# GATB/dsk

Measured on AMD Instinct MI355X. Metric: distinct k-mers counted/sec (whole node), k=31, higher is better.
Workload: dtype u64

## Files before the change

### dsk_amd/csrc/engine.h

```cpp
#pragma once
#include <algorithm>
#include <cstring>
#include <string>
#include <vector>

#include "../../include/dskgpu.h"
#include "layouts.h"

hipError_t placed_malloc(void** out, size_t bytes);

struct DevBuf {
    void* p = nullptr;
    size_t cap = 0;
    hipError_t ensure(size_t bytes) {
        if (bytes <= cap) return hipSuccess;
        size_t want = ((p ? bytes + bytes / 16 : bytes) + 255) & ~size_t(255);
        if (p) { (void)hipFree(p); p = nullptr; cap = 0; }
        hipError_t e = placed_malloc(&p, want);
        if (e == hipSuccess) cap = want; else p = nullptr;
        return e;
    }
    int ensure_keep(size_t bytes, size_t keep, hipStream_t stream) {
        if (bytes <= cap) return 0;
        void* np = nullptr;
        size_t want = ((std::max(bytes, cap + cap / 2) + 255) & ~size_t(255));
        if (hipMalloc(&np, want) != hipSuccess) return -1;
        if (keep && p) {
            if (hipMemcpyAsync(np, p, keep, hipMemcpyDeviceToDevice, stream) != hipSuccess || hipStreamSynchronize(stream) != hipSuccess) { (void)hipFree(np); return -1; }
        }
        if (p) (void)hipFree(p);
        p = np; cap = want;
        return 0;
    }
    void release() { if (p) (void)hipFree(p); p = nullptr; cap = 0; }
    template <class T> T* as() const { return reinterpret_cast<T*>(p); }
};

enum Scalar { SC_NCH1 = 0, SC_MLEN1, SC_NCH2, SC_MLEN2, SC_OVERFLOW, SC_F, SC_SORTFLAG, SC_OVF2, SC_OVF1, SC_RSLEN, SC_RSWORK, SC_RSWORK2, SC_RSTIES, SC_EXT, SC_NCHAINED, SC_NCH_S, SC_MLEN_S, SC_WORK2, SC_COUNT = 24 };

struct Stage { const char* name; hipEvent_t ev; };

struct Tuning {
    bool no_opt1 = false, no_opt2 = false;
    bool no_aligned = false;
    u32 rs_heavy = 0;
    u32 rs_bbits = 0;
    u32 rs_block_rows = 0;
    bool sk_exact = false, no_recsrc = false;
    u32 opt_cap = 0;
    u64 opt_slice = 0;
    u64 sk_slice = 0, sk_minslice = 2000;
    u32 table_maxload = 0;
    long long max_ext = -1;
    bool no_sample = false;
    bool no_heavy = false;
    bool verbose = false;
    bool no_level0 = false; u32 l0_passes = 0;
    u64 rs_max_rows = 0;
    u32 ps_maxc = 0;
    bool sk_generic = false;
    bool l0_keys = false;
    u32 mp_pass_mkeys = 0;
    u64 rs_slab_rows = 0;
    bool unitig_stages = false;
    bool cc_plain = false, cc_stages = false;
    bool correct_staged = false;
    void read() {
        auto on = [](const char* n) { return getenv(n) != nullptr; };
        auto num = [](const char* n, u64 dflt) { const char* e = getenv(n); return e ? (u64)atoll(e) : dflt; };
        no_opt1 = on("DSKGPU_NO_OPT1"); no_opt2 = on("DSKGPU_NO_OPT2"); no_aligned = on("DSKGPU_NO_ALIGNED");
        sk_exact = on("DSKGPU_SK_EXACT");
        no_recsrc = on("DSKGPU_NO_RECSRC");
        opt_cap = (u32)num("DSKGPU_OPT_CAP", 0) & ~7u; opt_slice = num("DSKGPU_OPT_SLICE", 0) & ~7ull;
        sk_slice = num("DSKGPU_SK_SLICE", 0); sk_minslice = num("DSKGPU_SK_MINSLICE", 2000);
        table_maxload = (u32)num("DSKGPU_TABLE_MAXLOAD", 0);
        max_ext = getenv("DSKGPU_MAX_EXT") ? atoll(getenv("DSKGPU_MAX_EXT")) : -1;
        no_sample = on("DSKGPU_NO_SAMPLE"); no_heavy = on("DSKGPU_NO_HEAVY"); verbose = on("DSKGPU_VERBOSE"); no_level0 = on("DSKGPU_NO_LEVEL0"); l0_passes = (u32)num("DSKGPU_L0_PASSES", 0); mp_pass_mkeys = (u32)num("DSKGPU_MP_PASS_MKEYS", 0); rs_max_rows = num("DSKGPU_RS_MAX_ROWS", 0); l0_keys = on("DSKGPU_L0_KEYS"); sk_generic = on("DSKGPU_SK_GENERIC"); ps_maxc = (u32)num("DSKGPU_PS_MAXC", 0);
        rs_slab_rows = num("DSKGPU_RS_SLAB_ROWS", 0);
        unitig_stages = on("DSKGPU_UNITIG_STAGES");
        cc_plain = on("DSKGPU_CC_PLAIN"); cc_stages = on("DSKGPU_CC_STAGES");
        correct_staged = on("DSKGPU_CORRECT_STAGED");
        rs_block_rows = (u32)num("DSKGPU_RS_BLOCK_ROWS", 0); rs_bbits = (u32)num("DSKGPU_RS_BBITS", 0); rs_heavy = (u32)num("DSKGPU_RS_HEAVY", 0);
    }
};

struct SparseRows {
    int W = 0;
    const void* keys = nullptr; const u32 *ab = nullptr, *soff = nullptr, *fstart = nullptr; u32 cap = 0, F = 0;
    u64 n_sparse = 0; u32 n_tail = 0; RowsIn tail_w{}; const u32* tail_ab = nullptr;
    template <class S> S as(u32 qpc = 0) const { return S{static_cast<decltype(S::keys)>(keys), ab, soff, fstart, cap, F, qpc}; }
    Rows2C tail2() const { return Rows2C{tail_w.w[1], tail_w.w[0], tail_ab}; }
};

struct PartPasses {
    struct Pass { u64 row_base; u32 nparts, off_index; };
    std::vector<Pass> passes; DevBuf part_off, flag; u32 off_used = 0; bool ok = false; u64 row_base = 0;
    std::vector<u32> h_off;
};

struct RowSort {
    DevBuf fix_list;
    DevBuf g[4];
    DevBuf del, lens;
    std::vector<u64> h_del; std::vector<u32> h_lens, h_lin;
    DevBuf ovs;
    u32 flag = 0, listed = 0;
    u64* hist_pin = nullptr; size_t hist_pin_n = 0;
    bool part_mode = false; u32 n_parts = 0; u32* h_part_off = nullptr; size_t h_part_cap = 0; DevBuf part_off;
    std::vector<u64> h_part_off64;
    PartPasses mp;
    void release() {
        for (DevBuf* b : {&fix_list, &g[0], &g[1], &g[2], &g[3], &del, &lens, &ovs, &part_off, &mp.part_off, &mp.flag}) b->release();
        if (hist_pin) (void)hipHostFree(hist_pin);
        if (h_part_off) (void)hipHostFree(h_part_off);
        hist_pin = nullptr; h_part_off = nullptr;
    }
};

struct Query {
    DevBuf table, packed, inval, deg;
    u64 cap = 0;
    bool valid = false;
    void release() { table.release(); packed.release(); inval.release(); deg.release(); cap = 0; valid = false; }
    void invalidate() { valid = false; }
};

struct Components {
    DevBuf comp, first, cols;
    dskgpu_component_stats stats{};
    bool valid = false;
    void release() { for (DevBuf* b : {&comp, &first, &cols}) b->release(); stats = dskgpu_component_stats{}; valid = false; }
// ... 237 lines not shown
```

### dsk_amd/csrc/partsort.h

```cpp
#pragma once
#include "rowsort.h"
#include "rowsort2.h"

#ifndef PS_NT
#define PS_NT 1024
#define PS_RPT 4
#endif
#define PS_CAP (PS_NT * PS_RPT)
#define PS_BINS 4096
#define PS_MAXC 4096u
#define PS_MAXQ 512

struct PsParams { u32 qpp, nparts_sparse; int sh; u32 n_tail, maxc; };

__global__ __launch_bounds__(PS_NT) void k_part_sort(RsSparse s, const u64* __restrict__ tail_k, const u32* __restrict__ tail_v, PsParams pp,
                                                     u64* __restrict__ ov, u32* __restrict__ oab, u32* __restrict__ part_off, u32* __restrict__ flag) {
    __shared__ u64 lk[PS_CAP];
    __shared__ u32 la[PS_CAP];
    __shared__ u32 cnt[PS_BINS];
    __shared__ u32 lsoff[PS_MAXQ + 1];
    __shared__ u32 wsum[PS_NT / 64 + 1];
    const u32 tid = threadIdx.x, lane = tid & 63, wave = tid >> 6;
    const u32 p = blockIdx.x;
    const bool is_tail = p >= pp.nparts_sparse;
    const u32 q0 = is_tail ? s.F : p * pp.qpp, q1 = is_tail ? s.F : (q0 + pp.qpp < s.F ? q0 + pp.qpp : s.F), nq = q1 - q0;
    for (u32 x = tid; x <= nq; x += PS_NT) lsoff[x] = s.soff[q0 + x];
    for (u32 b = tid; b < PS_BINS; b += PS_NT) cnt[b] = 0;
    __syncthreads();
    const u32 r0 = is_tail ? s.soff[s.F] : lsoff[0];
    const u32 n = is_tail ? pp.n_tail : lsoff[nq] - r0;
    if (tid == 0) {
        part_off[p] = r0;
        if (p + 1 == gridDim.x) part_off[p + 1] = r0 + n;
    }
    if (n > PS_CAP) {
        if (tid == 0) *flag = 1u;
        for (u32 i = tid; i < n; i += PS_NT) {
            const u32 r = r0 + i;
            if (is_tail) { ov[(u64)r] = tail_k[i]; oab[(u64)r] = tail_v[i]; }
            else {
                u32 lo = 0, hi = nq;
                while (hi - lo > 1) { const u32 mid = (lo + hi) >> 1; if (lsoff[mid] <= r) lo = mid; else hi = mid; }
                const u64 src = rs_sp_base(s, q0 + lo) + (u64)(r - lsoff[lo]);
                ov[(u64)r] = kunmix(s.keys[src]); oab[(u64)r] = s.ab[src];
            }
        }
        return;
    }
    if (n == 0) return;
    u64 k[PS_RPT]; u32 a[PS_RPT], rb[PS_RPT];
#pragma unroll
    for (int j = 0; j < PS_RPT; ++j) {
        const u32 i = tid + (u32)j * PS_NT;
        const u32 r = r0 + (i < n ? i : n - 1);
        if (is_tail) { k[j] = tail_k[r - r0]; a[j] = tail_v[r - r0]; }
        else {
            u32 lo = 0, hi = nq;
            while (hi - lo > 1) { const u32 mid = (lo + hi) >> 1; if (lsoff[mid] <= r) lo = mid; else hi = mid; }
            const u64 src = rs_sp_base(s, q0 + lo) + (u64)(r - lsoff[lo]);
            k[j] = kunmix(s.keys[src]); a[j] = s.ab[src];
        }
    }
#pragma unroll
    for (int j = 0; j < PS_RPT; ++j) {
        const u32 i = tid + (u32)j * PS_NT;
        u32 bin = (u32)(k[j] >> pp.sh); bin = bin < PS_BINS ? bin : PS_BINS - 1;
        rb[j] = i < n ? (bin << 16) | atomicAdd(&cnt[bin], 1u) : 0xFFFFFFFFu;
    }
    __syncthreads();
    {
        constexpr int CPT = PS_BINS / PS_NT;
        u32 c[CPT], sum = 0;
#pragma unroll
        for (int x = 0; x < CPT; ++x) { c[x] = cnt[tid * CPT + x]; sum += c[x]; }
        const u32 inc = wave_incl_scan(sum);
        if (lane == 63) wsum[wave] = inc;
        __syncthreads();
        u32 run = inc - sum;
#pragma unroll
        for (int x = 0; x < PS_NT / 64; ++x) { const u32 v = wsum[x]; if ((u32)x < wave) run += v; }
        bool heavy = false;
#pragma unroll
        for (int x = 0; x < CPT; ++x) { cnt[tid * CPT + x] = (run << 16) | c[x]; run += c[x]; heavy = heavy || c[x] > pp.maxc; }
        if (heavy) *flag = 1u;
    }
    __syncthreads();
    u32 pos[PS_RPT], cb[PS_RPT];
#pragma unroll
    for (int j = 0; j < PS_RPT; ++j) {
        pos[j] = 0; cb[j] = 0;
        if (rb[j] != 0xFFFFFFFFu) {
            cb[j] = cnt[rb[j] >> 16];
            pos[j] = (cb[j] >> 16) + (rb[j] & 0xFFFFu);
            lk[pos[j]] = k[j]; la[pos[j]] = a[j];
        }
    }
    __syncthreads();
    bool moved = false;
#pragma unroll
    for (int j = 0; j < PS_RPT; ++j) {
        const u32 c = cb[j] & 0xFFFFu;
        if (rb[j] != 0xFFFFFFFFu && c > 1u && c <= PS_MAXC) {
            const u32 o = cb[j] >> 16;
            u32 less = 0;
            for (u32 x = 0; x < c; ++x) less += lk[o + x] < k[j] ? 1u : 0u;
            pos[j] = o + less; moved = true;
        }
    }
    __syncthreads();
    if (moved) {
#pragma unroll
        for (int j = 0; j < PS_RPT; ++j)
            if (rb[j] != 0xFFFFFFFFu && (cb[j] & 0xFFFFu) > 1u && (cb[j] & 0xFFFFu) <= PS_MAXC) { lk[pos[j]] = k[j]; la[pos[j]] = a[j]; }
    }
    __syncthreads();
    for (u32 i = tid; i < n; i += PS_NT) { ov[(u64)r0 + i] = lk[i]; oab[(u64)r0 + i] = la[i]; }
}

#ifndef PS2_RPT
#define PS2_RPT 2
#endif
#define PS2_CAP (PS_NT * PS2_RPT)
__device__ __forceinline__ u32 ps2_bin(u64 hi, u64 lo, int sh) {
    const u64 v = sh >= 64 ? hi >> (sh - 64) : sh == 0 ? lo : ((hi << (64 - sh)) | (lo >> sh));
    return v < PS_BINS ? (u32)v : PS_BINS - 1;
}
__global__ __launch_bounds__(PS_NT) void k_part_sort2(Rs2Sparse s, Rows2C tail, PsParams pp, Rows2 o, u32* __restrict__ part_off, u32* __restrict__ flag) {
    __shared__ u64 lh[PS2_CAP];
    __shared__ u64 ll[PS2_CAP];
    __shared__ u32 la[PS2_CAP];
    __shared__ u32 cnt[PS_BINS];
    __shared__ u32 lsoff[PS_MAXQ + 1];
    __shared__ u32 wsum[PS_NT / 64 + 1];
    const u32 tid = threadIdx.x, lane = tid & 63, wave = tid >> 6;
    const u32 p = blockIdx.x;
    const bool is_tail = p >= pp.nparts_sparse;
    const u32 q0 = is_tail ? s.F : p * pp.qpp, q1 = is_tail ? s.F : (q0 + pp.qpp < s.F ? q0 + pp.qpp : s.F), nq = q1 - q0;
    for (u32 x = tid; x <= nq; x += PS_NT) lsoff[x] = s.soff[q0 + x];
    for (u32 b = tid; b < PS_BINS; b += PS_NT) cnt[b] = 0;
    __syncthreads();
    const u32 r0 = is_tail ? s.soff[s.F] : lsoff[0];
    const u32 n = is_tail ? pp.n_tail : lsoff[nq] - r0;
    if (tid == 0) {
        part_off[p] = r0;
        if (p + 1 == gridDim.x) part_off[p + 1] = r0 + n;
    }
    if (n > PS2_CAP) {
        if (tid == 0) *flag = 1u;
        for (u32 i = tid; i < n; i += PS_NT) {
            const u32 r = r0 + i;
            if (is_tail) { const u64 th = tail.hi[i], tl = tail.lo[i]; const u32 ta = tail.ab[i]; o.hi[(u64)r] = th; o.lo[(u64)r] = tl; o.ab[(u64)r] = ta; }
            else {
                u32 lo = 0, hi = nq;
                while (hi - lo > 1) { const u32 mid = (lo + hi) >> 1; if (lsoff[mid] <= r) lo = mid; else hi = mid; }
                const u64 src = rs2_sp_base(s, q0 + lo) + (u64)(r - lsoff[lo]);
                K2 kx = s.keys[src]; kunmixN(kx);
                o.hi[(u64)r] = kx.w[1]; o.lo[(u64)r] = kx.w[0]; o.ab[(u64)r] = s.ab[src];
            }
        }
        return;
    }
    if (n == 0) return;
    u64 kh[PS2_RPT], kl[PS2_RPT]; u32 a[PS2_RPT], rb[PS2_RPT];
#pragma unroll
    for (int j = 0; j < PS2_RPT; ++j) {
        const u32 i = tid + (u32)j * PS_NT;
        const u32 r = r0 + (i < n ? i : n - 1);
        if (is_tail) { kh[j] = tail.hi[r - r0]; kl[j] = tail.lo[r - r0]; a[j] = tail.ab[r - r0]; }
        else {
            u32 lo = 0, hi = nq;
            while (hi - lo > 1) { const u32 mid = (lo + hi) >> 1; if (lsoff[mid] <= r) lo = mid; else hi = mid; }
            const u64 src = rs2_sp_base(s, q0 + lo) + (u64)(r - lsoff[lo]);
            K2 kx = s.keys[src]; kunmixN(kx);
            kh[j] = kx.w[1]; kl[j] = kx.w[0]; a[j] = s.ab[src];
        }
    }
#pragma unroll
    for (int j = 0; j < PS2_RPT; ++j) {
        const u32 i = tid + (u32)j * PS_NT;
        const u32 bin = ps2_bin(kh[j], kl[j], pp.sh);
        rb[j] = i < n ? (bin << 16) | atomicAdd(&cnt[bin], 1u) : 0xFFFFFFFFu;
    }
    __syncthreads();
    {
        constexpr int CPT = PS_BINS / PS_NT;
        u32 c[CPT], sum = 0;
#pragma unroll
        for (int x = 0; x < CPT; ++x) { c[x] = cnt[tid * CPT + x]; sum += c[x]; }
        const u32 inc = wave_incl_scan(sum);
        if (lane == 63) wsum[wave] = inc;
        __syncthreads();
        u32 run = inc - sum;
#pragma unroll
        for (int x = 0; x < PS_NT / 64; ++x) { const u32 v = wsum[x]; if ((u32)x < wave) run += v; }
        bool heavy = false;
#pragma unroll
        for (int x = 0; x < CPT; ++x) { cnt[tid * CPT + x] = (run << 16) | c[x]; run += c[x]; heavy = heavy || c[x] > pp.maxc; }
        if (heavy) *flag = 1u;
    }
    __syncthreads();
    u32 pos[PS2_RPT], cb[PS2_RPT];
#pragma unroll
    for (int j = 0; j < PS2_RPT; ++j) {
        pos[j] = 0; cb[j] = 0;
        if (rb[j] != 0xFFFFFFFFu) {
            cb[j] = cnt[rb[j] >> 16];
            pos[j] = (cb[j] >> 16) + (rb[j] & 0xFFFFu);
            lh[pos[j]] = kh[j]; ll[pos[j]] = kl[j]; la[pos[j]] = a[j];
        }
    }
    __syncthreads();
    bool moved = false;
#pragma unroll
    for (int j = 0; j < PS2_RPT; ++j) {
        const u32 c = cb[j] & 0xFFFFu;
        if (rb[j] != 0xFFFFFFFFu && c > 1u && c <= PS_MAXC) {
            const u32 ob = cb[j] >> 16;
            u32 less = 0;
            for (u32 x = 0; x < c; ++x) { const u64 h = lh[ob + x], l = ll[ob + x]; less += (h < kh[j] || (h == kh[j] && l < kl[j])) ? 1u : 0u; }
            pos[j] = ob + less; moved = true;
        }
    }
    __syncthreads();
    if (moved) {
#pragma unroll
        for (int j = 0; j < PS2_RPT; ++j)
            if (rb[j] != 0xFFFFFFFFu && (cb[j] & 0xFFFFu) > 1u && (cb[j] & 0xFFFFu) <= PS_MAXC) { lh[pos[j]] = kh[j]; ll[pos[j]] = kl[j]; la[pos[j]] = a[j]; }
    }
    __syncthreads();
    for (u32 i = tid; i < n; i += PS_NT) { o.hi[(u64)r0 + i] = lh[i]; o.lo[(u64)r0 + i] = ll[i]; o.ab[(u64)r0 + i] = la[i]; }
}

#define PS4_CAP PS_NT
__device__ __forceinline__ u64 rs4_sp_base(const Rs4Sparse& s, u32 q) { return s.cap ? (u64)q * s.cap : (u64)s.fstart[q]; }
__device__ __forceinline__ u32 ps4_bin(u64 w0, u64 w1, u64 w2, u64 w3, int sh) {
    const int wi = sh >> 6, b = sh & 63;
    const u64 lo = wi == 0 ? w0 : wi == 1 ? w1 : wi == 2 ? w2 : w3;
    const u64 hi = wi == 0 ? w1 : wi == 1 ? w2 : wi == 2 ? w3 : 0ull;
    const u64 v = b ? (lo >> b) | (hi << (64 - b)) : lo;
    return v < PS_BINS ? (u32)v : PS_BINS - 1;
}
__global__ __launch_bounds__(PS_NT) void k_part_sort4(Rs4Sparse s, PsParams pp, RowsOut o, u32* oab, u32* part_off, u32* flag) {
    __shared__ u64 lw[4][PS4_CAP];
    __shared__ u32 la[PS4_CAP];
    __shared__ u32 cnt[PS_BINS];
    __shared__ u32 lsoff[PS_MAXQ + 1];
    __shared__ u32 wsum[PS_NT / 64 + 1];
    const u32 tid = threadIdx.x, lane = tid & 63, wave = tid >> 6;
    const u32 p = blockIdx.x;
    const u32 q0 = p * pp.qpp < s.F ? p * pp.qpp : s.F, q1 = q0 + pp.qpp < s.F ? q0 + pp.qpp : s.F, nq = q1 - q0;
    for (u32 x = tid; x <= nq; x += PS_NT) lsoff[x] = s.soff[q0 + x];
    for (u32 b = tid; b < PS_BINS; b += PS_NT) cnt[b] = 0;
    __syncthreads();
    const u32 r0 = lsoff[0];
    const u32 n = lsoff[nq] - r0;
    if (tid == 0) {
        part_off[p] = r0;
        if (p + 1 == gridDim.x) part_off[p + 1] = r0 + n;
    }
    if (n > PS4_CAP) {
        if (tid == 0) *flag = 1u;
        for (u32 i = tid; i < n; i += PS_NT) {
            const u32 r = r0 + i;
            u32 lo = 0, hi = nq;
            while (hi - lo > 1) { const u32 mid = (lo + hi) >> 1; if (lsoff[mid] <= r) lo = mid; else hi = mid; }
            const u64 src = rs4_sp_base(s, q0 + lo) + (u64)(r - lsoff[lo]);
            KN<4> kx;
#pragma unroll
            for (int x = 0; x < 4; ++x) kx.w[x] = s.keys[src].w[x];
            kunmixN(kx);
#pragma unroll
            for (int x = 0; x < 4; ++x) o.w[x][(u64)r] = kx.w[x];
            oab[(u64)r] = s.ab[src];
        }
        return;
    }
    if (n == 0) return;
    const bool have = tid < n;
    u64 k0, k1, k2, k3; u32 a;
    {
        const u32 r = r0 + (have ? tid : n - 1);
        u32 lo = 0, hi = nq;
        while (hi - lo > 1) { const u32 mid = (lo + hi) >> 1; if (lsoff[mid] <= r) lo = mid; else hi = mid; }
// ... 56 lines not shown
```

### dsk_amd/csrc/rowsort.hip

```cpp
#include <cstdio>
#include <vector>

#include "engine.h"
#include "partsort.h"

#include <rocprim/device/device_radix_sort.hpp>

namespace {

__global__ void k_set_rs_scalars(u32* __restrict__ sc4, u32 len, u32 nwords, u32* __restrict__ z0 = nullptr, u32* __restrict__ z1 = nullptr) {
    if (threadIdx.x == 0) sc4[0] = len;
    else if (threadIdx.x < nwords) sc4[threadIdx.x] = 0u;
    if (threadIdx.x == 32 && z0) *z0 = 0u;
    if (threadIdx.x == 33 && z1) *z1 = 0u;
}
__global__ void k_sort_back(const u32* __restrict__ sc, const u32* __restrict__ ovs, u64* __restrict__ out) {
    if (threadIdx.x == 0) { out[0] = sc[SC_SORTFLAG]; out[1] = ovs ? ovs[0] : 0u; }
}
#ifndef SORT_TOP_BITS
#define SORT_TOP_BITS 32u
#endif

template <class T>
int grow_pinned(dskgpu_ctx* ctx, T*& p, size_t& cap, size_t need, size_t alloc) {
// ... 531 lines not shown
                { const int e2 = rows2_rounds(ctx, r2, s2); if (e2) return e2; }
            }
            lib = ctx->rs.flag != 0;
        }
        if (lib && m >= 0xFFFF0000ull) return fail(ctx, DSKGPU_E_OVERFLOW, "row sort: one value range of the >= 2^32 rows holds 2^32 rows itself (not a k-mer spectrum)");
        if (lib && W == 2) {
            const u64* src[2] = {T.lo + b, T.hi + b};
            { const int rc = sort_index_multiword(ctx, src, m, 2); if (rc) return rc; }
            const unsigned gb = (unsigned)((m + 255) / 256);
            const u32* idx = ctx->srt_idx.as<u32>();
            hipLaunchKernelGGL(k_gather<u64>, dim3(gb), dim3(256), 0, ctx->stream, K.lo + b, (const u64*)(T.lo + b), idx, m);
            hipLaunchKernelGGL(k_gather<u64>, dim3(gb), dim3(256), 0, ctx->stream, K.hi + b, (const u64*)(T.hi + b), idx, m);
            hipLaunchKernelGGL(k_gather<u32>, dim3(gb), dim3(256), 0, ctx->stream, K.ab + b, (const u32*)(T.ab + b), idx, m);
            CKL("row sort: group gather");
            CK(hipMemcpyAsync(T.lo + b, K.lo + b, m * 8, hipMemcpyDeviceToDevice, ctx->stream));
            CK(hipMemcpyAsync(T.hi + b, K.hi + b, m * 8, hipMemcpyDeviceToDevice, ctx->stream));
            CK(hipMemcpyAsync(T.ab + b, K.ab + b, m * 4, hipMemcpyDeviceToDevice, ctx->stream));
            CK(hipStreamSynchronize(ctx->stream));
            ctx->stats.sort_fallback = 1; ++nlib;
        } else if (lib) {
            size_t tmp = 0;
            const unsigned end_bit = (unsigned)(total - sb);
            CK(rocprim::radix_sort_pairs(nullptr, tmp, tk + b, k + b, tv + b, v + b, (size_t)m, 0u, end_bit, ctx->stream));
            CK(ctx->srt_tmp.ensure(tmp));
            CK(rocprim::radix_sort_pairs(ctx->srt_tmp.p, tmp, tk + b, k + b, tv + b, v + b, (size_t)m, 0u, end_bit, ctx->stream));
            CK(hipMemcpyAsync(tk + b, k + b, m * 8, hipMemcpyDeviceToDevice, ctx->stream));
            CK(hipMemcpyAsync(tv + b, v + b, m * 4, hipMemcpyDeviceToDevice, ctx->stream));
            CK(hipStreamSynchronize(ctx->stream));
            ctx->stats.sort_fallback = 1; ++nlib;
        }
    }
    if (ctx->tune.verbose) fprintf(stderr, "[dskgpu] row sort: %llu rows (>= 2^32 path) in %u slab(s), %u group(s) on their top %d bits, %u through the library sort\n", (unsigned long long)n, S, ngroups, sb, nlib);
    ctx->rs.flag = 0; ctx->rs.listed = 0;
    if (W == 1) { ctx->res_w[0] = tk; ctx->res_ab = tv; }
    else { ctx->res_w[1] = T.hi; ctx->res_w[0] = T.lo; ctx->res_ab = T.ab; }
    return DSKGPU_OK;
}

}

static u64 part_sort_cap(int W) { return W == 1 ? PS_CAP : W == 2 ? PS2_CAP : PS4_CAP; }
static u32 part_sort_qpp(int W, u64 F, u64 n_sparse) {
    const u64 mean = std::max<u64>(1, (n_sparse + F - 1) / std::max<u64>(F, 1));
    return (u32)std::min<u64>(std::max<u64>(1, (part_sort_cap(W) * 3 / 4) / mean), PS_MAXQ);
}
u32 part_sort_nparts(const SparseRows& rows) {
    const u32 qpp = part_sort_qpp(rows.W, rows.F, rows.n_sparse);
    return (u32)((rows.F + qpp - 1) / qpp) + (rows.n_tail ? 1u : 0u);
}
int launch_part_sort(dskgpu_ctx* ctx, const SparseRows& rows, RowsOut out, u32* out_ab, u32* d_part_off, u32* d_flag, u32* nparts_out) {
    const int W = rows.W;
    const u32 qpp = part_sort_qpp(W, rows.F, rows.n_sparse), nparts = part_sort_nparts(rows), nps = nparts - (rows.n_tail ? 1u : 0u);
    const int sh = std::max(0, 2 * (int)ctx->cfg.kmer_size - 12);
    const PsParams pp{qpp, nps, W == 1 ? std::min(sh, 52) : sh, rows.n_tail, ctx->tune.ps_maxc ? std::min<u32>(ctx->tune.ps_maxc, PS_MAXC) : PS_MAXC};
    if (W == 1) hipLaunchKernelGGL(k_part_sort, dim3(nparts), dim3(PS_NT), 0, ctx->stream, rows.as<RsSparse>(), rows.tail_w.w[0], rows.tail_ab, pp, out.w[0], out_ab, d_part_off, d_flag);
    else if (W == 2) hipLaunchKernelGGL(k_part_sort2, dim3(nparts), dim3(PS_NT), 0, ctx->stream, rows.as<Rs2Sparse>(), rows.tail2(), pp, Rows2{out.w[1], out.w[0], out_ab}, d_part_off, d_flag);
    else hipLaunchKernelGGL(k_part_sort4, dim3(nparts), dim3(PS_NT), 0, ctx->stream, rows.as<Rs4Sparse>(), pp, out, out_ab, d_part_off, d_flag);
    CKL("k_part_sort");
    *nparts_out = nparts;
    return DSKGPU_OK;
}

namespace {

int sort_rows_partition_order(dskgpu_ctx* ctx, const SparseRows& rows, u64 n, Round* r) {
    const int W = rows.W;
    const u32 nparts = part_sort_nparts(rows);
    DevBuf* dst_w = W == 4 ? ctx->out_w : ctx->srt_w;
    DevBuf& dst_ab = W == 4 ? ctx->out_ab : ctx->srt_ab;
    for (int x = 0; x < W; ++x) CK(dst_w[x].ensure(n * 8));
    CK(dst_ab.ensure(n * 4));
    CK(ctx->rs.part_off.ensure(((size_t)nparts + 2) * 4));
    { const int rc = grow_pinned(ctx, ctx->rs.h_part_off, ctx->rs.h_part_cap, (size_t)nparts + 2, ((size_t)nparts + 2) * 2); if (rc) return rc; }
    u32* sc = ctx->scalars.as<u32>();
    hipLaunchKernelGGL(k_set_rs_scalars, dim3(1), dim3(64), 0, ctx->stream, sc + SC_RSLEN, 0u, 1u, sc + SC_SORTFLAG, (u32*)nullptr);
    u32 np = 0;
    RowsOut out{};
    for (int x = 0; x < W; ++x) out.w[x] = dst_w[x].as<u64>();
    { const int rc = launch_part_sort(ctx, rows, out, dst_ab.as<u32>(), ctx->rs.part_off.as<u32>(), sc + SC_SORTFLAG, &np); if (rc) return rc; }
    CK(hipMemcpyAsync(ctx->rs.h_part_off, ctx->rs.part_off.p, ((size_t)nparts + 1) * 4, hipMemcpyDeviceToHost, ctx->stream));
    ctx->rs.part_mode = true; ctx->rs.n_parts = nparts; ctx->rs.h_part_off64.clear();
    r->back = 2;
    for (int x = 0; x < W; ++x) ctx->res_w[x] = dst_w[x].as<u64>();
    ctx->res_ab = dst_ab.as<u32>();
    return DSKGPU_OK;
}

int sort_rows4(dskgpu_ctx* ctx, u64 n, Round* r) {
    constexpr int W = 4;
    CK(ctx->srt_k.ensure(n * 8)); CK(ctx->s_val.ensure(n * 8));
    CK(ctx->srt_idx.ensure(n * 4)); CK(ctx->srt_idx2.ensure(n * 4));
    const unsigned gb = (unsigned)((n + 255) / 256);
    RowsIn ri{}; RowsOut ro{};
    for (int x = 0; x < W; ++x) { CK(ctx->srt_w[x].ensure(n * 8)); ri.w[x] = ctx->out_w[x].as<u64>(); ro.w[x] = ctx->srt_w[x].as<u64>(); }
    const int bits = 2 * (int)ctx->cfg.kmer_size;
    const bool msd = n <= RS_MAX_ROWS;
    u64* aos = nullptr;
    if (msd) {
        CK(ctx->srt_k2.ensure(n * 8 * (size_t)AosRow<W>::WORDS));
        aos = ctx->srt_k2.as<u64>();
        hipLaunchKernelGGL(k_top_key_aos<W>, dim3(gb), dim3(256), 0, ctx->stream, ri, ctx->out_ab.as<u32>(), n, bits, ctx->srt_k.as<u64>(), ctx->srt_idx.as<u32>(), aos);
    } else hipLaunchKernelGGL(k_top_key<W>, dim3(gb), dim3(256), 0, ctx->stream, ri, n, bits, ctx->srt_k.as<u64>(), ctx->srt_idx.as<u32>());
    u32* flag = ctx->scalars.as<u32>() + SC_SORTFLAG;
    const u32* ties = nullptr;
    const u32* idx; const u64* skey; int run_shift;
    if (msd) {
        const int e = msd_sort_pairs(ctx, ctx->srt_k.as<u64>(), ctx->srt_idx.as<u32>(), ctx->s_val.as<u64>(), ctx->srt_idx2.as<u32>(), n, 63);
        if (e) return e;
        CK(hipMemcpyAsync(&ctx->rs.flag, flag, 4, hipMemcpyDeviceToHost, ctx->stream));
// ... 156 lines not shown
```

Measured before the change: 27.02 billion.

## Make partition sort persistent with prefetch of next partition's rows

Converts k_part_sort and k_part_sort2 into persistent kernels launched with a grid of about two blocks per CU. Each block loops over partitions with stride gridDim and double-buffers the segment offsets. The global loads for the next partition are issued while the current one is binned and sorted in shared memory. This targets the load latency that each block previously exposed before any compute, at the cost of more registers, extra synchronisation, and less occupancy-driven latency hiding. A DSKGPU_PS_GRID env knob sets the grid size.

```diff
diff --git a/dsk_amd/csrc/engine.h b/dsk_amd/csrc/engine.h
--- a/dsk_amd/csrc/engine.h
+++ b/dsk_amd/csrc/engine.h
@@ -58,6 +58,7 @@
     bool no_level0 = false; u32 l0_passes = 0;
     u64 rs_max_rows = 0;
     u32 ps_maxc = 0;
+    u32 ps_grid = 0;
     bool sk_generic = false;
     bool l0_keys = false;
     u32 mp_pass_mkeys = 0;
@@ -77,6 +78,7 @@
         max_ext = getenv("DSKGPU_MAX_EXT") ? atoll(getenv("DSKGPU_MAX_EXT")) : -1;
         no_sample = on("DSKGPU_NO_SAMPLE"); no_heavy = on("DSKGPU_NO_HEAVY"); verbose = on("DSKGPU_VERBOSE"); no_level0 = on("DSKGPU_NO_LEVEL0"); l0_passes = (u32)num("DSKGPU_L0_PASSES", 0); mp_pass_mkeys = (u32)num("DSKGPU_MP_PASS_MKEYS", 0); rs_max_rows = num("DSKGPU_RS_MAX_ROWS", 0); l0_keys = on("DSKGPU_L0_KEYS"); sk_generic = on("DSKGPU_SK_GENERIC"); ps_maxc = (u32)num("DSKGPU_PS_MAXC", 0);
         rs_slab_rows = num("DSKGPU_RS_SLAB_ROWS", 0);
+        ps_grid = (u32)std::min<u64>(num("DSKGPU_PS_GRID", 0), 1u << 20);
         unitig_stages = on("DSKGPU_UNITIG_STAGES");
         cc_plain = on("DSKGPU_CC_PLAIN"); cc_stages = on("DSKGPU_CC_STAGES");
         correct_staged = on("DSKGPU_CORRECT_STAGED");
diff --git a/dsk_amd/csrc/partsort.h b/dsk_amd/csrc/partsort.h
--- a/dsk_amd/csrc/partsort.h
+++ b/dsk_amd/csrc/partsort.h
@@ -11,110 +11,153 @@
 #define PS_MAXC 4096u
 #define PS_MAXQ 512
 
-struct PsParams { u32 qpp, nparts_sparse; int sh; u32 n_tail, maxc; };
+struct PsParams { u32 qpp, nparts_sparse; int sh; u32 n_tail, maxc, nblocks; };
 
-__global__ __launch_bounds__(PS_NT) void k_part_sort(RsSparse s, const u64* __restrict__ tail_k, const u32* __restrict__ tail_v, PsParams pp,
+__device__ __forceinline__ u32 ps_q0(const PsParams& pp, u32 F, u32 p) { return p >= pp.nparts_sparse ? F : p * pp.qpp; }
+__device__ __forceinline__ u32 ps_nq(const PsParams& pp, u32 F, u32 p) {
+    if (p >= pp.nparts_sparse) return 0u;
+    const u32 q0 = p * pp.qpp;
+    return (q0 + pp.qpp < F ? q0 + pp.qpp : F) - q0;
+}
+__global__ __launch_bounds__(PS_NT, 8) void k_part_sort(RsSparse s, const u64* __restrict__ tail_k, const u32* __restrict__ tail_v, PsParams pp,
                                                      u64* __restrict__ ov, u32* __restrict__ oab, u32* __restrict__ part_off, u32* __restrict__ flag) {
     __shared__ u64 lk[PS_CAP];
     __shared__ u32 la[PS_CAP];
     __shared__ u32 cnt[PS_BINS];
-    __shared__ u32 lsoff[PS_MAXQ + 1];
+    __shared__ u32 lsoff[2][PS_MAXQ + 1];
     __shared__ u32 wsum[PS_NT / 64 + 1];
     const u32 tid = threadIdx.x, lane = tid & 63, wave = tid >> 6;
-    const u32 p = blockIdx.x;
-    const bool is_tail = p >= pp.nparts_sparse;
-    const u32 q0 = is_tail ? s.F : p * pp.qpp, q1 = is_tail ? s.F : (q0 + pp.qpp < s.F ? q0 + pp.qpp : s.F), nq = q1 - q0;
-    for (u32 x = tid; x <= nq; x += PS_NT) lsoff[x] = s.soff[q0 + x];
+    const u32 G = gridDim.x;
+    u32 p = blockIdx.x;
+    if (p >= pp.nblocks) return;
+    u64 kn[PS_RPT]; u32 an[PS_RPT];
+#pragma unroll
+    for (int j = 0; j < PS_RPT; ++j) { kn[j] = 0; an[j] = 0; }
+    auto fetch = [&](u32 pf, const u32* ls) {
+        const bool tl = pf >= pp.nparts_sparse;
+        const u32 q0 = ps_q0(pp, s.F, pf), nq = ps_nq(pp, s.F, pf);
+        const u32 r0 = ls[0], n = tl ? pp.n_tail : ls[nq] - r0;
+        if (n == 0 || n > PS_CAP) return;
+#pragma unroll
+        for (int j = 0; j < PS_RPT; ++j) {
+            const u32 i = tid + (u32)j * PS_NT;
+            const u32 ii = i < n ? i : n - 1;
+            if (tl) { kn[j] = tail_k[ii]; an[j] = tail_v[ii]; }
+            else {
+                const u32 r = r0 + ii;
+                u32 lo = 0, hi = nq;
+                while (hi - lo > 1) { const u32 mid = (lo + hi) >> 1; if (ls[mid] <= r) lo = mid; else hi = mid; }
+                const u64 src = rs_sp_base(s, q0 + lo) + (u64)(r - ls[lo]);
+                kn[j] = s.keys[src]; an[j] = s.ab[src];
+            }
+        }
+    };
     for (u32 b = tid; b < PS_BINS; b += PS_NT) cnt[b] = 0;
-    __syncthreads();
-    const u32 r0 = is_tail ? s.soff[s.F] : lsoff[0];
-    const u32 n = is_tail ? pp.n_tail : lsoff[nq] - r0;
-    if (tid == 0) {
-        part_off[p] = r0;
-        if (p + 1 == gridDim.x) part_off[p + 1] = r0 + n;
-    }
-    if (n > PS_CAP) {
-        if (tid == 0) *flag = 1u;
-        for (u32 i = tid; i < n; i += PS_NT) {
-            const u32 r = r0 + i;
-            if (is_tail) { ov[(u64)r] = tail_k[i]; oab[(u64)r] = tail_v[i]; }
-            else {
-                u32 lo = 0, hi = nq;
-                while (hi - lo > 1) { const u32 mid = (lo + hi) >> 1; if (lsoff[mid] <= r) lo = mid; else hi = mid; }
-                const u64 src = rs_sp_base(s, q0 + lo) + (u64)(r - lsoff[lo]);
-                ov[(u64)r] = kunmix(s.keys[src]); oab[(u64)r] = s.ab[src];
-            }
-        }
-        return;
-    }
-    if (n == 0) return;
-    u64 k[PS_RPT]; u32 a[PS_RPT], rb[PS_RPT];
-#pragma unroll
-    for (int j = 0; j < PS_RPT; ++j) {
-        const u32 i = tid + (u32)j * PS_NT;
-        const u32 r = r0 + (i < n ? i : n - 1);
-        if (is_tail) { k[j] = tail_k[r - r0]; a[j] = tail_v[r - r0]; }
-        else {
-            u32 lo = 0, hi = nq;
-            while (hi - lo > 1) { const u32 mid = (lo + hi) >> 1; if (lsoff[mid] <= r) lo = mid; else hi = mid; }
-            const u64 src = rs_sp_base(s, q0 + lo) + (u64)(r - lsoff[lo]);
-            k[j] = kunmix(s.keys[src]); a[j] = s.ab[src];
-        }
-    }
-#pragma unroll
-    for (int j = 0; j < PS_RPT; ++j) {
-        const u32 i = tid + (u32)j * PS_NT;
-        u32 bin = (u32)(k[j] >> pp.sh); bin = bin < PS_BINS ? bin : PS_BINS - 1;
-        rb[j] = i < n ? (bin << 16) | atomicAdd(&cnt[bin], 1u) : 0xFFFFFFFFu;
-    }
-    __syncthreads();
-    {
-        constexpr int CPT = PS_BINS / PS_NT;
-        u32 c[CPT], sum = 0;
-#pragma unroll
-        for (int x = 0; x < CPT; ++x) { c[x] = cnt[tid * CPT + x]; sum += c[x]; }
-        const u32 inc = wave_incl_scan(sum);
-        if (lane == 63) wsum[wave] = inc;
+    if (tid <= ps_nq(pp, s.F, p)) lsoff[0][tid] = s.soff[ps_q0(pp, s.F, p) + tid];
+    __syncthreads();
+    fetch(p, lsoff[0]);
+    u32 so = 0;
+    if (p + G < pp.nblocks && tid <= ps_nq(pp, s.F, p + G)) so = s.soff[ps_q0(pp, s.F, p + G) + tid];
+    for (u32 cur = 0;; cur ^= 1u) {
+        const u32 pn = p + G;
+        const bool has_next = pn < pp.nblocks;
+        const u32* ls = lsoff[cur];
+        u32* lsn = lsoff[cur ^ 1u];
+        if (has_next && tid <= ps_nq(pp, s.F, pn)) lsn[tid] = so;
+        const bool is_tail = p >= pp.nparts_sparse;
+        const u32 q0 = ps_q0(pp, s.F, p), nq = ps_nq(pp, s.F, p);
+        const u32 r0 = ls[0];
+        const u32 n = is_tail ? pp.n_tail : ls[nq] - r0;
+        const bool ordered = n != 0 && n <= PS_CAP;
+        if (tid == 0) {
+            part_off[p] = r0;
+            if (p + 1 == pp.nblocks) part_off[p + 1] = r0 + n;
+        }
+        u64 k[PS_RPT]; u32 a[PS_RPT], rb[PS_RPT];
+        if (ordered) {
+#pragma unroll
+            for (int j = 0; j < PS_RPT; ++j) {
+                const u32 i = tid + (u32)j * PS_NT;
+                k[j] = is_tail ? kn[j] : kunmix(kn[j]); a[j] = an[j];
+                u32 bin = (u32)(k[j] >> pp.sh); bin = bin < PS_BINS ? bin : PS_BINS - 1;
+                rb[j] = i < n ? (bin << 16) | atomicAdd(&cnt[bin], 1u) : 0xFFFFFFFFu;
+            }
+        }
         __syncthreads();
-        u32 run = inc - sum;
-#pragma unroll
-        for (int x = 0; x < PS_NT / 64; ++x) { const u32 v = wsum[x]; if ((u32)x < wave) run += v; }
-        bool heavy = false;
-#pragma unroll
-        for (int x = 0; x < CPT; ++x) { cnt[tid * CPT + x] = (run << 16) | c[x]; run += c[x]; heavy = heavy || c[x] > pp.maxc; }
-        if (heavy) *flag = 1u;
-    }
-    __syncthreads();
-    u32 pos[PS_RPT], cb[PS_RPT];
-#pragma unroll
-    for (int j = 0; j < PS_RPT; ++j) {
-        pos[j] = 0; cb[j] = 0;
-        if (rb[j] != 0xFFFFFFFFu) {
-            cb[j] = cnt[rb[j] >> 16];
-            pos[j] = (cb[j] >> 16) + (rb[j] & 0xFFFFu);
-            lk[pos[j]] = k[j]; la[pos[j]] = a[j];
-        }
-    }
-    __syncthreads();
-    bool moved = false;
-#pragma unroll
-    for (int j = 0; j < PS_RPT; ++j) {
-        const u32 c = cb[j] & 0xFFFFu;
-        if (rb[j] != 0xFFFFFFFFu && c > 1u && c <= PS_MAXC) {
-            const u32 o = cb[j] >> 16;
-            u32 less = 0;
-            for (u32 x = 0; x < c; ++x) less += lk[o + x] < k[j] ? 1u : 0u;
-            pos[j] = o + less; moved = true;
-        }
-    }
-    __syncthreads();
-    if (moved) {
-#pragma unroll
-        for (int j = 0; j < PS_RPT; ++j)
-            if (rb[j] != 0xFFFFFFFFu && (cb[j] & 0xFFFFu) > 1u && (cb[j] & 0xFFFFu) <= PS_MAXC) { lk[pos[j]] = k[j]; la[pos[j]] = a[j]; }
-    }
-    __syncthreads();
-    for (u32 i = tid; i < n; i += PS_NT) { ov[(u64)r0 + i] = lk[i]; oab[(u64)r0 + i] = la[i]; }
+        if (has_next) {
+            fetch(pn, lsn);
+            if (pn + G < pp.nblocks && tid <= ps_nq(pp, s.F, pn + G)) so = s.soff[ps_q0(pp, s.F, pn + G) + tid];
+        }
+        if (n > PS_CAP) {
+            if (tid == 0) *flag = 1u;
+            for (u32 i = tid; i < n; i += PS_NT) {
+                const u32 r = r0 + i;
+                if (is_tail) { ov[(u64)r] = tail_k[i]; oab[(u64)r] = tail_v[i]; }
+                else {
+                    u32 lo = 0, hi = nq;
+                    while (hi - lo > 1) { const u32 mid = (lo + hi) >> 1; if (ls[mid] <= r) lo = mid; else hi = mid; }
+                    const u64 src = rs_sp_base(s, q0 + lo) + (u64)(r - ls[lo]);
+                    ov[(u64)r] = kunmix(s.keys[src]); oab[(u64)r] = s.ab[src];
+                }
+            }
+        } else if (ordered) {
+            {
+                constexpr int CPT = PS_BINS / PS_NT;
+                u32 c[CPT], sum = 0;
+#pragma unroll
+                for (int x = 0; x < CPT; ++x) { c[x] = cnt[tid * CPT + x]; sum += c[x]; }
+                const u32 inc = wave_incl_scan(sum);
+                if (lane == 63) wsum[wave] = inc;
+                __syncthreads();
+                u32 run = inc - sum;
+#pragma unroll
+                for (int x = 0; x < PS_NT / 64; ++x) { const u32 v = wsum[x]; if ((u32)x < wave) run += v; }
+                bool heavy = false;
+#pragma unroll
+                for (int x = 0; x < CPT; ++x) { cnt[tid * CPT + x] = (run << 16) | c[x]; run += c[x]; heavy = heavy || c[x] > pp.maxc; }
+                if (heavy) *flag = 1u;
+            }
+            __syncthreads();
+            u32 pos[PS_RPT], cb[PS_RPT];
+#pragma unroll
+            for (int j = 0; j < PS_RPT; ++j) {
+                pos[j] = 0; cb[j] = 0;
+                if (rb[j] != 0xFFFFFFFFu) {
+                    cb[j] = cnt[rb[j] >> 16];
+                    pos[j] = (cb[j] >> 16) + (rb[j] & 0xFFFFu);
+                    lk[pos[j]] = k[j]; la[pos[j]] = a[j];
+                }
+            }
+            __syncthreads();
+            for (u32 b = tid; b < PS_BINS; b += PS_NT) cnt[b] = 0;
+            bool moved = false;
+#pragma unroll
+            for (int j = 0; j < PS_RPT; ++j) {
+                const u32 c = cb[j] & 0xFFFFu;
+                if (rb[j] != 0xFFFFFFFFu && c > 1u && c <= PS_MAXC) {
+                    const u32 o = cb[j] >> 16;
+                    u32 less = 0;
+                    for (u32 x = 0; x < c; ++x) less += lk[o + x] < k[j] ? 1u : 0u;
+                    pos[j] = o + less; moved = true;
+                }
+            }
+            __syncthreads();
+            if (moved) {
+#pragma unroll
+                for (int j = 0; j < PS_RPT; ++j)
+                    if (rb[j] != 0xFFFFFFFFu && (cb[j] & 0xFFFFu) > 1u && (cb[j] & 0xFFFFu) <= PS_MAXC) { lk[pos[j]] = k[j]; la[pos[j]] = a[j]; }
+            }
+            __syncthreads();
+#pragma unroll
+            for (int j = 0; j < PS_RPT; ++j) {
+                const u32 i = tid + (u32)j * PS_NT;
+                if (i < n) { ov[(u64)r0 + i] = lk[i]; oab[(u64)r0 + i] = la[i]; }
+            }
+        }
+        if (!has_next) break;
+        __syncthreads();
+        p = pn;
+    }
 }
 
 #ifndef PS2_RPT
@@ -125,110 +168,149 @@
     const u64 v = sh >= 64 ? hi >> (sh - 64) : sh == 0 ? lo : ((hi << (64 - sh)) | (lo >> sh));
     return v < PS_BINS ? (u32)v : PS_BINS - 1;
 }
-__global__ __launch_bounds__(PS_NT) void k_part_sort2(Rs2Sparse s, Rows2C tail, PsParams pp, Rows2 o, u32* __restrict__ part_off, u32* __restrict__ flag) {
+__global__ __launch_bounds__(PS_NT, 8) void k_part_sort2(Rs2Sparse s, Rows2C tail, PsParams pp, Rows2 o, u32* __restrict__ part_off, u32* __restrict__ flag) {
     __shared__ u64 lh[PS2_CAP];
     __shared__ u64 ll[PS2_CAP];
     __shared__ u32 la[PS2_CAP];
     __shared__ u32 cnt[PS_BINS];
-    __shared__ u32 lsoff[PS_MAXQ + 1];
+    __shared__ u32 lsoff[2][PS_MAXQ + 1];
     __shared__ u32 wsum[PS_NT / 64 + 1];
     const u32 tid = threadIdx.x, lane = tid & 63, wave = tid >> 6;
-    const u32 p = blockIdx.x;
-    const bool is_tail = p >= pp.nparts_sparse;
-    const u32 q0 = is_tail ? s.F : p * pp.qpp, q1 = is_tail ? s.F : (q0 + pp.qpp < s.F ? q0 + pp.qpp : s.F), nq = q1 - q0;
-    for (u32 x = tid; x <= nq; x += PS_NT) lsoff[x] = s.soff[q0 + x];
+    const u32 G = gridDim.x;
+    u32 p = blockIdx.x;
+    if (p >= pp.nblocks) return;
+    u64 nh[PS2_RPT], nl[PS2_RPT]; u32 an[PS2_RPT];
+#pragma unroll
+    for (int j = 0; j < PS2_RPT; ++j) { nh[j] = 0; nl[j] = 0; an[j] = 0; }
+    auto fetch = [&](u32 pf, const u32* ls) {
+        const bool tl = pf >= pp.nparts_sparse;
+        const u32 q0 = ps_q0(pp, s.F, pf), nq = ps_nq(pp, s.F, pf);
+        const u32 r0 = ls[0], n = tl ? pp.n_tail : ls[nq] - r0;
+        if (n == 0 || n > PS2_CAP) return;
+#pragma unroll
+        for (int j = 0; j < PS2_RPT; ++j) {
+            const u32 i = tid + (u32)j * PS_NT;
+            const u32 ii = i < n ? i : n - 1;
+            if (tl) { nh[j] = tail.hi[ii]; nl[j] = tail.lo[ii]; an[j] = tail.ab[ii]; }
+            else {
+                const u32 r = r0 + ii;
+                u32 lo = 0, hi = nq;
+                while (hi - lo > 1) { const u32 mid = (lo + hi) >> 1; if (ls[mid] <= r) lo = mid; else hi = mid; }
+                const u64 src = rs2_sp_base(s, q0 + lo) + (u64)(r - ls[lo]);
+                const K2 kx = s.keys[src];
+                nh[j] = kx.w[1]; nl[j] = kx.w[0]; an[j] = s.ab[src];
+            }
+        }
+    };
     for (u32 b = tid; b < PS_BINS; b += PS_NT) cnt[b] = 0;
-    __syncthreads();
-    const u32 r0 = is_tail ? s.soff[s.F] : lsoff[0];
-    const u32 n = is_tail ? pp.n_tail : lsoff[nq] - r0;
-    if (tid == 0) {
-        part_off[p] = r0;
-        if (p + 1 == gridDim.x) part_off[p + 1] = r0 + n;
-    }
-    if (n > PS2_CAP) {
-        if (tid == 0) *flag = 1u;
-        for (u32 i = tid; i < n; i += PS_NT) {
-            const u32 r = r0 + i;
-            if (is_tail) { const u64 th = tail.hi[i], tl = tail.lo[i]; const u32 ta = tail.ab[i]; o.hi[(u64)r] = th; o.lo[(u64)r] = tl; o.ab[(u64)r] = ta; }
-            else {
-                u32 lo = 0, hi = nq;
-                while (hi - lo > 1) { const u32 mid = (lo + hi) >> 1; if (lsoff[mid] <= r) lo = mid; else hi = mid; }
-                const u64 src = rs2_sp_base(s, q0 + lo) + (u64)(r - lsoff[lo]);
-                K2 kx = s.keys[src]; kunmixN(kx);
-                o.hi[(u64)r] = kx.w[1]; o.lo[(u64)r] = kx.w[0]; o.ab[(u64)r] = s.ab[src];
-            }
-        }
-        return;
-    }
-    if (n == 0) return;
-    u64 kh[PS2_RPT], kl[PS2_RPT]; u32 a[PS2_RPT], rb[PS2_RPT];
-#pragma unroll
-    for (int j = 0; j < PS2_RPT; ++j) {
-        const u32 i = tid + (u32)j * PS_NT;
-        const u32 r = r0 + (i < n ? i : n - 1);
-        if (is_tail) { kh[j] = tail.hi[r - r0]; kl[j] = tail.lo[r - r0]; a[j] = tail.ab[r - r0]; }
-        else {
-            u32 lo = 0, hi = nq;
-            while (hi - lo > 1) { const u32 mid = (lo + hi) >> 1; if (lsoff[mid] <= r) lo = mid; else hi = mid; }
-            const u64 src = rs2_sp_base(s, q0 + lo) + (u64)(r - lsoff[lo]);
-            K2 kx = s.keys[src]; kunmixN(kx);
-            kh[j] = kx.w[1]; kl[j] = kx.w[0]; a[j] = s.ab[src];
-        }
-    }
-#pragma unroll
-    for (int j = 0; j < PS2_RPT; ++j) {
-        const u32 i = tid + (u32)j * PS_NT;
-        const u32 bin = ps2_bin(kh[j], kl[j], pp.sh);
-        rb[j] = i < n ? (bin << 16) | atomicAdd(&cnt[bin], 1u) : 0xFFFFFFFFu;
-    }
-    __syncthreads();
-    {
-        constexpr int CPT = PS_BINS / PS_NT;
-        u32 c[CPT], sum = 0;
-#pragma unroll
-        for (int x = 0; x < CPT; ++x) { c[x] = cnt[tid * CPT + x]; sum += c[x]; }
-        const u32 inc = wave_incl_scan(sum);
-        if (lane == 63) wsum[wave] = inc;
+    if (tid <= ps_nq(pp, s.F, p)) lsoff[0][tid] = s.soff[ps_q0(pp, s.F, p) + tid];
+    __syncthreads();
+    fetch(p, lsoff[0]);
+    u32 so = 0;
+    if (p + G < pp.nblocks && tid <= ps_nq(pp, s.F, p + G)) so = s.soff[ps_q0(pp, s.F, p + G) + tid];
+    for (u32 cur = 0;; cur ^= 1u) {
+        const u32 pn = p + G;
+        const bool has_next = pn < pp.nblocks;
+        const u32* ls = lsoff[cur];
+        u32* lsn = lsoff[cur ^ 1u];
+        if (has_next && tid <= ps_nq(pp, s.F, pn)) lsn[tid] = so;
+        const bool is_tail = p >= pp.nparts_sparse;
+        const u32 q0 = ps_q0(pp, s.F, p), nq = ps_nq(pp, s.F, p);
+        const u32 r0 = ls[0];
+        const u32 n = is_tail ? pp.n_tail : ls[nq] - r0;
+        const bool ordered = n != 0 && n <= PS2_CAP;
+        if (tid == 0) {
+            part_off[p] = r0;
+            if (p + 1 == pp.nblocks) part_off[p + 1] = r0 + n;
+        }
+        u64 kh[PS2_RPT], kl[PS2_RPT]; u32 a[PS2_RPT], rb[PS2_RPT];
+        if (ordered) {
+#pragma unroll
+            for (int j = 0; j < PS2_RPT; ++j) {
+                const u32 i = tid + (u32)j * PS_NT;
+                K2 kx; kx.w[1] = nh[j]; kx.w[0] = nl[j];
+                if (!is_tail) kunmixN(kx);
+                kh[j] = kx.w[1]; kl[j] = kx.w[0]; a[j] = an[j];
+                const u32 bin = ps2_bin(kh[j], kl[j], pp.sh);
+                rb[j] = i < n ? (bin << 16) | atomicAdd(&cnt[bin], 1u) : 0xFFFFFFFFu;
+            }
+        }
         __syncthreads();
-        u32 run = inc - sum;
-#pragma unroll
-        for (int x = 0; x < PS_NT / 64; ++x) { const u32 v = wsum[x]; if ((u32)x < wave) run += v; }
-        bool heavy = false;
-#pragma unroll
-        for (int x = 0; x < CPT; ++x) { cnt[tid * CPT + x] = (run << 16) | c[x]; run += c[x]; heavy = heavy || c[x] > pp.maxc; }
-        if (heavy) *flag = 1u;
-    }
-    __syncthreads();
-    u32 pos[PS2_RPT], cb[PS2_RPT];
-#pragma unroll
-    for (int j = 0; j < PS2_RPT; ++j) {
-        pos[j] = 0; cb[j] = 0;
-        if (rb[j] != 0xFFFFFFFFu) {
-            cb[j] = cnt[rb[j] >> 16];
-            pos[j] = (cb[j] >> 16) + (rb[j] & 0xFFFFu);
-            lh[pos[j]] = kh[j]; ll[pos[j]] = kl[j]; la[pos[j]] = a[j];
-        }
-    }
-    __syncthreads();
-    bool moved = false;
-#pragma unroll
-    for (int j = 0; j < PS2_RPT; ++j) {
-        const u32 c = cb[j] & 0xFFFFu;
-        if (rb[j] != 0xFFFFFFFFu && c > 1u && c <= PS_MAXC) {
-            const u32 ob = cb[j] >> 16;
-            u32 less = 0;
-            for (u32 x = 0; x < c; ++x) { const u64 h = lh[ob + x], l = ll[ob + x]; less += (h < kh[j] || (h == kh[j] && l < kl[j])) ? 1u : 0u; }
-            pos[j] = ob + less; moved = true;
-        }
-    }
-    __syncthreads();
-    if (moved) {
-#pragma unroll
-        for (int j = 0; j < PS2_RPT; ++j)
-            if (rb[j] != 0xFFFFFFFFu && (cb[j] & 0xFFFFu) > 1u && (cb[j] & 0xFFFFu) <= PS_MAXC) { lh[pos[j]] = kh[j]; ll[pos[j]] = kl[j]; la[pos[j]] = a[j]; }
-    }
-    __syncthreads();
-    for (u32 i = tid; i < n; i += PS_NT) { o.hi[(u64)r0 + i] = lh[i]; o.lo[(u64)r0 + i] = ll[i]; o.ab[(u64)r0 + i] = la[i]; }
+        if (has_next) {
+            fetch(pn, lsn);
+            if (pn + G < pp.nblocks && tid <= ps_nq(pp, s.F, pn + G)) so = s.soff[ps_q0(pp, s.F, pn + G) + tid];
+        }
+        if (n > PS2_CAP) {
+            if (tid == 0) *flag = 1u;
+            for (u32 i = tid; i < n; i += PS_NT) {
+                const u32 r = r0 + i;
+                if (is_tail) { const u64 th = tail.hi[i], tl = tail.lo[i]; const u32 ta = tail.ab[i]; o.hi[(u64)r] = th; o.lo[(u64)r] = tl; o.ab[(u64)r] = ta; }
+                else {
+                    u32 lo = 0, hi = nq;
+                    while (hi - lo > 1) { const u32 mid = (lo + hi) >> 1; if (ls[mid] <= r) lo = mid; else hi = mid; }
+                    const u64 src = rs2_sp_base(s, q0 + lo) + (u64)(r - ls[lo]);
+                    K2 kx = s.keys[src]; kunmixN(kx);
+                    o.hi[(u64)r] = kx.w[1]; o.lo[(u64)r] = kx.w[0]; o.ab[(u64)r] = s.ab[src];
+                }
+            }
+        } else if (ordered) {
+            {
+                constexpr int CPT = PS_BINS / PS_NT;
+                u32 c[CPT], sum = 0;
+#pragma unroll
+                for (int x = 0; x < CPT; ++x) { c[x] = cnt[tid * CPT + x]; sum += c[x]; }
+                const u32 inc = wave_incl_scan(sum);
+                if (lane == 63) wsum[wave] = inc;
+                __syncthreads();
+                u32 run = inc - sum;
+#pragma unroll
+                for (int x = 0; x < PS_NT / 64; ++x) { const u32 v = wsum[x]; if ((u32)x < wave) run += v; }
+                bool heavy = false;
+#pragma unroll
+                for (int x = 0; x < CPT; ++x) { cnt[tid * CPT + x] = (run << 16) | c[x]; run += c[x]; heavy = heavy || c[x] > pp.maxc; }
+                if (heavy) *flag = 1u;
+            }
+            __syncthreads();
+            u32 pos[PS2_RPT], cb[PS2_RPT];
+#pragma unroll
+            for (int j = 0; j < PS2_RPT; ++j) {
+                pos[j] = 0; cb[j] = 0;
+                if (rb[j] != 0xFFFFFFFFu) {
+                    cb[j] = cnt[rb[j] >> 16];
+                    pos[j] = (cb[j] >> 16) + (rb[j] & 0xFFFFu);
+                    lh[pos[j]] = kh[j]; ll[pos[j]] = kl[j]; la[pos[j]] = a[j];
+                }
+            }
+            __syncthreads();
+            for (u32 b = tid; b < PS_BINS; b += PS_NT) cnt[b] = 0;
+            bool moved = false;
+#pragma unroll
+            for (int j = 0; j < PS2_RPT; ++j) {
+                const u32 c = cb[j] & 0xFFFFu;
+                if (rb[j] != 0xFFFFFFFFu && c > 1u && c <= PS_MAXC) {
+                    const u32 ob = cb[j] >> 16;
+                    u32 less = 0;
+                    for (u32 x = 0; x < c; ++x) { const u64 h = lh[ob + x], l = ll[ob + x]; less += (h < kh[j] || (h == kh[j] && l < kl[j])) ? 1u : 0u; }
+                    pos[j] = ob + less; moved = true;
+                }
+            }
+            __syncthreads();
+            if (moved) {
+#pragma unroll
+                for (int j = 0; j < PS2_RPT; ++j)
+                    if (rb[j] != 0xFFFFFFFFu && (cb[j] & 0xFFFFu) > 1u && (cb[j] & 0xFFFFu) <= PS_MAXC) { lh[pos[j]] = kh[j]; ll[pos[j]] = kl[j]; la[pos[j]] = a[j]; }
+            }
+            __syncthreads();
+#pragma unroll
+            for (int j = 0; j < PS2_RPT; ++j) {
+                const u32 i = tid + (u32)j * PS_NT;
+                if (i < n) { o.hi[(u64)r0 + i] = lh[i]; o.lo[(u64)r0 + i] = ll[i]; o.ab[(u64)r0 + i] = la[i]; }
+            }
+        }
+        if (!has_next) break;
+        __syncthreads();
+        p = pn;
+    }
 }
 
 #define PS4_CAP PS_NT
diff --git a/dsk_amd/csrc/rowsort.hip b/dsk_amd/csrc/rowsort.hip
--- a/dsk_amd/csrc/rowsort.hip
+++ b/dsk_amd/csrc/rowsort.hip
@@ -607,9 +607,10 @@
     const int W = rows.W;
     const u32 qpp = part_sort_qpp(W, rows.F, rows.n_sparse), nparts = part_sort_nparts(rows), nps = nparts - (rows.n_tail ? 1u : 0u);
     const int sh = std::max(0, 2 * (int)ctx->cfg.kmer_size - 12);
-    const PsParams pp{qpp, nps, W == 1 ? std::min(sh, 52) : sh, rows.n_tail, ctx->tune.ps_maxc ? std::min<u32>(ctx->tune.ps_maxc, PS_MAXC) : PS_MAXC};
-    if (W == 1) hipLaunchKernelGGL(k_part_sort, dim3(nparts), dim3(PS_NT), 0, ctx->stream, rows.as<RsSparse>(), rows.tail_w.w[0], rows.tail_ab, pp, out.w[0], out_ab, d_part_off, d_flag);
-    else if (W == 2) hipLaunchKernelGGL(k_part_sort2, dim3(nparts), dim3(PS_NT), 0, ctx->stream, rows.as<Rs2Sparse>(), rows.tail2(), pp, Rows2{out.w[1], out.w[0], out_ab}, d_part_off, d_flag);
+    const PsParams pp{qpp, nps, W == 1 ? std::min(sh, 52) : sh, rows.n_tail, ctx->tune.ps_maxc ? std::min<u32>(ctx->tune.ps_maxc, PS_MAXC) : PS_MAXC, nparts};
+    const u32 grid = std::min<u32>(nparts, ctx->tune.ps_grid ? ctx->tune.ps_grid : 2u * (u32)ctx->num_cu);
+    if (W == 1) hipLaunchKernelGGL(k_part_sort, dim3(grid), dim3(PS_NT), 0, ctx->stream, rows.as<RsSparse>(), rows.tail_w.w[0], rows.tail_ab, pp, out.w[0], out_ab, d_part_off, d_flag);
+    else if (W == 2) hipLaunchKernelGGL(k_part_sort2, dim3(grid), dim3(PS_NT), 0, ctx->stream, rows.as<Rs2Sparse>(), rows.tail2(), pp, Rows2{out.w[1], out.w[0], out_ab}, d_part_off, d_flag);
     else hipLaunchKernelGGL(k_part_sort4, dim3(nparts), dim3(PS_NT), 0, ctx->stream, rows.as<Rs4Sparse>(), pp, out, out_ab, d_part_off, d_flag);
     CKL("k_part_sort");
     *nparts_out = nparts;
```

Result: no change. 26.95 billion (-0.3%).
